# DavidPetrus/ood_object_detection

Hardware: AMD Instinct MI355X
Metric: images/sec, tf_efficientdet_d0 640px bf16 inference + OOD score (DetBenchPredict end-to-end) (higher is better)
Workload: dtype bf16; 1 GPU; tf_efficientdet_d0 640x640 batch=64/GPU C=90, DetBenchPredict: backbone+BiFPN+heads+OOD energy/max-logit+top-k(5000)+decode+hard NMS; global_batch=64, parallelism=image-sharded dp1, no collective, weights=seeded reference init, randomised BN stats, class bias 0, launch=hipgraph, images_in_flight=192

## Files before the change

### include/effdet_hip.h

```cpp
#ifndef EFFDET_HIP_H
#define EFFDET_HIP_H

#ifdef __cplusplus
extern "C" {
#endif

#define EFFDET_F32 0
#define EFFDET_BF16 1
#define EFFDET_BF16X2 2
#define EFFDET_PAD_SYMMETRIC (1 << 24)

int effdet_abi_version(void);
const char* effdet_last_error(void);
int effdet_device_error(int clear);


int effdet_stem_conv(void* stream, int in_dtype, int out_dtype, const void* X, const float* Wt,
                     const float* scale, const float* shift, void* Y, int B, int H, int W, int Cout);

int effdet_stem_dw_fused(void* stream, int in_dtype, int dtype, const void* X, const void* Wk,
                         const float* s1, const float* t1, const float* taps, const float* s2, const float* t2,
                         void* Y, float* pool_partial, int B, int H, int W, int C);
int effdet_stem_dw_parts(int dtype, int H, int W, int C);

int effdet_resize_pad_u8(void* stream, const unsigned char* src, int h, int w, unsigned char* dst, int S, int sw, int sh,
                         const int* bounds_x, const int* coef_x, int ksize_x,
                         const int* bounds_y, const int* coef_y, int ksize_y,
                         const int* fill_rgb, unsigned char* workspace);
int effdet_normalize_u8(void* stream, int out_dtype, const unsigned char* X, const float* mean, const float* stdv,
                        void* Y, int B, int C, long long hw);

typedef struct EffdetResampleDesc {
    const unsigned char* src;
    int h, w;
    int flip_h, flip_v;
    int cx0, cy0, cw, ch;
    int filter;
    int sw, sh;
    int ox, oy;
    int reserved;
} EffdetResampleDesc;
int effdet_resample_batch_u8(void* stream, const EffdetResampleDesc* desc, const EffdetResampleDesc* desc_host, int B,
                             unsigned char* dst, long long dst_image_stride, int S, const int* fill_rgb);

typedef struct EffdetBoxParams {
    float img_w, img_h;
    int flip_h, flip_v;
    float pre_y, pre_x, scale, post_y, post_x, clip_h, clip_w;
    int reserved;
} EffdetBoxParams;
int effdet_transform_boxes(void* stream, const float* boxes, const long long* classes, const EffdetBoxParams* params,
                           int B, int Mmax, float* out_boxes, long long* out_classes, int* counts, unsigned char* valid);
int effdet_stem_conv_u8(void* stream, int out_dtype, const unsigned char* X, const float* mean, const float* stdv,
                        const float* Wt, const float* scale, const float* shift, void* Y, int B, int H, int W, int Cout);
int effdet_stem_dw_fused_u8(void* stream, int dtype, const unsigned char* X, const float* mean, const float* stdv,
                            const void* Wk, const float* s1, const float* t1, const float* taps, const float* s2, const float* t2,
                            void* Y, float* pool_partial, int B, int H, int W, int C);

int effdet_pw_gemm_bn_act(void* stream, int dtype, const void* A, long long M, int K, const void* W, int N,
                          const float* scale, const float* shift, int act, const void* residual,
                          const float* gate, int rows_per_image,
                          void* C, long long c_image_stride, long long ldc);
int effdet_pw_gemm_group(void* stream, int dtype, int n, const void* const* A, const long long* M, const int* K,
                         const void* const* W, const int* N, const float* const* scale, const float* const* shift,
                         int act, void* const* C);

int effdet_dwconv_bn_act(void* stream, int dtype, const void* X, void* Y, const float* Wt,
                         const float* scale, const float* shift, int act, float* pool_partial,
                         int B, int H, int W, int C, int k, int stride);
int effdet_dwconv_blocks_per_image(int Ho, int Wo, int C);

int effdet_mbconv_expand_dw(void* stream, int dtype, const void* X, void* Y, const void* W1,
                            const float* s1, const float* t1, const float* taps,
                            const float* s2, const float* t2, float* pool_partial,
                            int B, int H, int W, int Cin, int mid, int k, int stride);
int effdet_mbconv_tiles_per_image(int dtype, int H, int W, int Cin, int mid, int k, int stride);
int effdet_mbconv_expand_dw_gated(void* stream, int dtype, const void* X, const float* in_gate, void* Y, const void* W1,
                                  const float* s1, const float* t1, const float* taps,
                                  const float* s2, const float* t2, float* pool_partial,
                                  int B, int H, int W, int Cin, int mid, int k, int stride);
int effdet_mbconv_gated_tiles_per_image(int dtype, int H, int W, int Cin, int mid, int k, int stride);
#define EFFDET_MBCONV_PLAN_INTS 17
int effdet_mbconv_plan_describe(int dtype, int H, int W, int Cin, int mid, int k, int stride, int gated, int* out, int n);

int effdet_se_gate(void* stream, const float* partial, int nblk, int hw, const float* W1, const float* b1,
                   const float* W2t, const float* b2, float* gate, int B, int C, int R);


int effdet_maxpool_same(void* stream, int dtype, const void* X, long long x_image_stride,
                        void* Y, long long y_image_stride, int B, int H, int W, int C);

int effdet_sepconv_fused(void* stream, int dtype, int B, int nlevels, const int* level_hw, int n_in,
                         const void* const* in_ptr, const long long* in_image_stride, const int* in_hw,
                         const int* in_mode, int fuse_mode, const float* fuse_w, float fuse_den, int pre_act,
                         const float* dw_w, const void* pw_w, const float* scale, const float* shift,
                         const int* affine_row, int post_act, int F, int N,
                         void* const* out_ptr, const long long* out_image_stride,
                         int ood_classes, int num_anchors, float* ood_energy, float* ood_maxlogit,
                         long long ood_image_stride, const long long* ood_level_off);

int effdet_sepconv_meta(void* stream, int dtype, int B, int nlevels, const int* level_hw,
                        const void* const* in_ptr, const long long* in_image_stride,
                        const float* in_scale, const float* in_shift, const int* in_affine_row, int pre_act,
                        const float* dw_w, const void* pw_w, const float* bias, int F, int N,
                        void* const* out_ptr, const long long* out_image_stride,
                        float* stat_partial, void* const* dw_out, const long long* dw_out_image_stride);
int effdet_sepconv_tiles(int dtype, int nlevels, const int* level_hw, int* level_tile_begin);
int effdet_bn_batch_stats(void* stream, int dtype, const float* partial, int B, int nlevels, const int* level_hw, int N,
                          const float* weight, const float* bias, const int* param_row, float eps,
                          float* out_scale, float* out_shift);


long long effdet_topk_workspace_bytes(int B, long long n_anchors);
int effdet_topk_select(void* stream, int dtype, const void* cls_all, const float* anchor_max, int B, long long n_anchors, int C,
                       const void* box_all, int k, void* out_cls, void* out_box,
                       long long* out_indices, long long* out_classes, void* workspace, long long workspace_bytes);

int effdet_decode_threshold(void* stream, int dtype, const void* cls_topk, const void* box_topk,
                            const float* anchors, const long long* indices, const long long* classes,
                            const float* img_scale, const float* img_size, int B, int k,
                            float* boxes, float* scores, int* classes_out, int* src, int* count, float* maxcoord);
int effdet_decode_threshold_gather(void* stream, int dtype, const void* cls_topk, const void* box_all, long long n_anchors,
                                   const float* anchors, const long long* indices, const long long* classes,
                                   const float* img_scale, const float* img_size, int B, int k,
                                   float* boxes, float* scores, int* classes_out, int* src, int* count, float* maxcoord);

int effdet_nms_hard(void* stream, const float* boxes, const float* scores, const int* classes, const int* src,
                    const int* count, const float* maxcoord, int B, int k, double iou_threshold, int max_det,
                    const float* img_scale, float* det, int* det_count, int* keep_src);

int effdet_detections_hard(void* stream, int dtype, const void* cls_topk, const void* box, long long n_anchors,
                           const float* anchors, const long long* indices, const long long* classes,
                           const float* img_scale_clip, const float* img_size, int B, int k,
                           float* boxes, float* scores, int* classes_out, int* src, int* count, float* maxcoord,
                           double iou_threshold, int max_det, const float* img_scale_out,
                           float* det, int* det_count, int* keep_src);

int effdet_nms_soft(void* stream, const float* boxes, const float* scores, const int* classes, const int* src,
                    const int* count, const float* maxcoord, int B, int k, int method_gaussian, float sigma,
                    float iou_threshold, float score_threshold, int max_det,
                    const float* img_scale, float* det, int* det_count, int* keep_src);

int effdet_nms_soft_large(void* stream, const float* boxes, const float* scores, const int* classes, const int* src,
                          const int* count, const float* maxcoord, int B, int k, int method_gaussian, float sigma,
                          float iou_threshold, float score_threshold, int max_det,
// ... 345 lines not shown
```

### ood_object_detection_amd/_lib.py

```python
import ctypes
import os
import subprocess

_HERE = os.path.dirname(os.path.abspath(__file__))
LIB_PATH = os.path.join(_HERE, 'libeffdet_hip.so')
CSRC = os.path.join(_HERE, 'csrc')

_lib = None

LABEL_PAD = -2 ** 63

c_void_p, c_int, c_ll, c_float, c_double = ctypes.c_void_p, ctypes.c_int, ctypes.c_longlong, ctypes.c_float, ctypes.c_double
P = ctypes.POINTER

SIGNATURES = {
    'effdet_abi_version': (c_int, []),
    'effdet_last_error': (ctypes.c_char_p, []),
    'effdet_device_error': (c_int, [c_int]),
    'effdet_stem_conv': (c_int, [c_void_p, c_int, c_int, c_void_p, c_void_p, c_void_p, c_void_p, c_void_p,
                                 c_int, c_int, c_int, c_int]),
    'effdet_stem_dw_fused': (c_int, [c_void_p, c_int, c_int, c_void_p, c_void_p, c_void_p, c_void_p, c_void_p, c_void_p,
                                     c_void_p, c_void_p, c_void_p, c_int, c_int, c_int, c_int]),
    'effdet_resize_pad_u8': (c_int, [c_void_p, c_void_p, c_int, c_int, c_void_p, c_int, c_int, c_int, c_void_p, c_void_p, c_int,
                                     c_void_p, c_void_p, c_int, c_void_p, c_void_p]),
    'effdet_resample_batch_u8': (c_int, [c_void_p, c_void_p, c_void_p, c_int, c_void_p, c_ll, c_int, c_void_p]),
    'effdet_transform_boxes': (c_int, [c_void_p, c_void_p, c_void_p, c_void_p, c_int, c_int, c_void_p, c_void_p, c_void_p, c_void_p]),
    'effdet_normalize_u8': (c_int, [c_void_p, c_int, c_void_p, c_void_p, c_void_p, c_void_p, c_int, c_int, c_ll]),
    'effdet_stem_conv_u8': (c_int, [c_void_p, c_int, c_void_p, c_void_p, c_void_p, c_void_p, c_void_p, c_void_p, c_void_p,
                                    c_int, c_int, c_int, c_int]),
    'effdet_stem_dw_fused_u8': (c_int, [c_void_p, c_int, c_void_p, c_void_p, c_void_p, c_void_p, c_void_p, c_void_p, c_void_p,
                                        c_void_p, c_void_p, c_void_p, c_void_p, c_int, c_int, c_int, c_int]),
    'effdet_stem_dw_parts': (c_int, [c_int, c_int, c_int, c_int]),
    'effdet_pw_gemm_bn_act': (c_int, [c_void_p, c_int, c_void_p, c_ll, c_int, c_void_p, c_int, c_void_p, c_void_p,
                                      c_int, c_void_p, c_void_p, c_int, c_void_p, c_ll, c_ll]),
    'effdet_pw_gemm_group': (c_int, [c_void_p, c_int, c_int, P(c_void_p), P(c_ll), P(c_int), P(c_void_p), P(c_int), P(c_void_p),
                                     P(c_void_p), c_int, P(c_void_p)]),
    'effdet_dwconv_bn_act': (c_int, [c_void_p, c_int, c_void_p, c_void_p, c_void_p, c_void_p, c_void_p, c_int,
                                     c_void_p, c_int, c_int, c_int, c_int, c_int, c_int]),
    'effdet_dwconv_blocks_per_image': (c_int, [c_int, c_int, c_int]),
    'effdet_mbconv_gated_tiles_per_image': (c_int, [c_int, c_int, c_int, c_int, c_int, c_int, c_int]),
    'effdet_mbconv_expand_dw_gated': (c_int, [c_void_p, c_int, c_void_p, c_void_p, c_void_p, c_void_p, c_void_p, c_void_p, c_void_p,
                                              c_void_p, c_void_p, c_void_p, c_int, c_int, c_int, c_int, c_int, c_int, c_int]),
    'effdet_mbconv_expand_dw': (c_int, [c_void_p, c_int, c_void_p, c_void_p, c_void_p, c_void_p, c_void_p, c_void_p,
                                        c_void_p, c_void_p, c_void_p, c_int, c_int, c_int, c_int, c_int, c_int, c_int]),
    'effdet_mbconv_tiles_per_image': (c_int, [c_int, c_int, c_int, c_int, c_int, c_int, c_int]),
    'effdet_mbconv_plan_describe': (c_int, [c_int, c_int, c_int, c_int, c_int, c_int, c_int, c_int, P(c_int), c_int]),
    'effdet_se_gate': (c_int, [c_void_p, c_void_p, c_int, c_int, c_void_p, c_void_p, c_void_p, c_void_p,
                               c_void_p, c_int, c_int, c_int]),
    'effdet_maxpool_same': (c_int, [c_void_p, c_int, c_void_p, c_ll, c_void_p, c_ll, c_int, c_int, c_int, c_int]),
    'effdet_sepconv_fused': (c_int, [c_void_p, c_int, c_int, c_int, P(c_int), c_int,
                                     P(c_void_p), P(c_ll), P(c_int), P(c_int), c_int, P(c_float), c_float, c_int,
                                     c_void_p, c_void_p, c_void_p, c_void_p, P(c_int), c_int, c_int, c_int,
                                     P(c_void_p), P(c_ll), c_int, c_int, c_void_p, c_void_p, c_ll, P(c_ll)]),
    'effdet_weighted_median': (c_int, [c_void_p, c_void_p, c_void_p, c_int, c_int, c_void_p, c_void_p]),
    'effdet_sqnorm_workspace_floats': (c_ll, []),
    'effdet_sqnorm': (c_int, [c_void_p, c_void_p, c_ll, c_void_p, c_void_p, c_int]),
    'effdet_adam_clip_step': (c_int, [c_void_p, c_void_p, c_void_p, c_void_p, c_void_p, c_ll, c_float, c_float, c_float, c_float,
                                      c_int, c_float, c_void_p]),
    'effdet_adam_clip_step_dev': (c_int, [c_void_p, c_void_p, c_void_p, c_void_p, c_void_p, c_ll, c_float, c_float, c_float, c_float,
                                          c_void_p, c_float, c_void_p]),
    'effdet_group_piece_floats': (c_ll, []),
    'effdet_group_norms': (c_int, [c_void_p, c_void_p, c_ll, c_void_p, c_int, c_int, c_void_p, c_int, c_void_p, c_int, c_void_p, c_int,
                                   c_void_p, c_void_p]),
    'effdet_group_step': (c_int, [c_void_p, c_int, c_void_p, c_void_p, c_void_p, c_void_p, c_ll, c_void_p, c_int, c_int, c_void_p, c_int,
                                  c_void_p, c_int, c_void_p, c_int, c_void_p, c_void_p, c_void_p, c_void_p]),
    'effdet_novelty_score': (c_int, [c_void_p, c_void_p, c_void_p, c_void_p, c_int, c_int, c_int, c_float, c_float, c_int,
                                     c_void_p, c_void_p, c_void_p]),
    'effdet_ood_image_score': (c_int, [c_void_p, c_void_p, c_int, c_ll, c_void_p]),
    'effdet_auroc_counts': (c_int, [c_void_p, c_void_p, c_void_p, c_int, c_int, c_void_p]),
    'effdet_ood_eval_workspace_bytes': (c_ll, [c_ll, c_ll]),
    'effdet_ood_eval_sort_tile': (c_int, []),
    'effdet_ood_eval_sorted_offset': (c_ll, [c_ll, c_ll, c_int]),
    'effdet_ood_eval_append': (c_int, [c_void_p, c_void_p, c_ll, c_ll, c_int, c_int, c_void_p, c_int, c_void_p, c_ll, c_ll, c_float,
                                       c_int, c_void_p, c_ll, c_void_p, c_void_p, c_ll]),
    'effdet_ood_eval_sort': (c_int, [c_void_p, c_void_p, c_ll, c_void_p, c_ll, c_void_p, c_void_p, c_ll]),
    'effdet_ood_eval_metrics': (c_int, [c_void_p, c_ll, c_ll, c_void_p, c_void_p, c_ll, c_double, c_void_p]),
    'effdet_feature_ood_workspace_bytes': (c_ll, [c_ll, c_int]),
    'effdet_feature_ood_fit': (c_int, [c_void_p, c_int, c_int, P(c_void_p), P(c_ll), P(c_ll), P(c_ll), P(c_ll), c_int, c_int, c_int, c_int,
                                       c_ll, c_void_p, c_void_p, c_int, c_ll, c_ll, c_ll, c_void_p, c_int, c_void_p, c_void_p, c_void_p,
                                       c_void_p, c_ll]),
    'effdet_feature_ood_score': (c_int, [c_void_p, c_int, c_int, P(c_void_p), P(c_ll), P(c_ll), P(c_ll), P(c_ll), c_int, c_int, c_int,
                                         c_int, c_ll, c_void_p, c_void_p, c_int, c_void_p, c_void_p, c_void_p, c_void_p, c_void_p,
                                         c_void_p, c_void_p, c_void_p]),
    'effdet_feature_knn_workspace_bytes': (c_ll, [c_ll, c_int, c_int, c_int]),
    'effdet_feature_knn_append': (c_int, [c_void_p, c_int, c_int, P(c_void_p), P(c_ll), P(c_ll), P(c_ll), P(c_ll), c_int, c_int, c_int, c_int,
                                          c_ll, c_void_p, c_void_p, c_int, c_ll, c_ll, c_ll, c_void_p, c_int, c_int, c_ll, c_ll, c_void_p,
                                          c_void_p, c_void_p, c_void_p, c_void_p, c_ll]),
    'effdet_feature_knn_score': (c_int, [c_void_p, c_int, c_int, P(c_void_p), P(c_ll), P(c_ll), P(c_ll), P(c_ll), c_int, c_int, c_int,
                                         c_ll, c_void_p, c_void_p, c_int, c_int, c_int, c_int, c_ll, c_void_p, c_void_p, c_void_p,
                                         c_void_p, c_void_p, c_void_p, c_void_p, c_ll]),
    'effdet_feature_subspace_score': (c_int, [c_void_p, c_int, c_int, P(c_void_p), P(c_ll), P(c_ll), P(c_ll), P(c_ll), c_int, c_int, c_int,
                                              c_ll, c_void_p, c_void_p, c_int, c_void_p, c_void_p, c_void_p, c_int, c_void_p, c_ll, c_ll,
                                              c_int, c_float, c_void_p, c_void_p, c_void_p]),
    'effdet_feature_subspace_calibrate': (c_int, [c_void_p, c_int, c_int, P(c_void_p), P(c_ll), P(c_ll), P(c_ll), P(c_ll), c_int, c_int,
                                                  c_int, c_ll, c_void_p, c_void_p, c_int, c_void_p, c_void_p, c_int, c_void_p, c_ll, c_ll,
                                                  c_int, c_void_p, c_void_p, c_void_p, c_ll]),
    'effdet_feature_subspace_workspace_bytes': (c_ll, [c_ll]),
    'effdet_logit_ood_score': (c_int, [c_void_p, c_int, c_void_p, c_ll, c_ll, c_int, c_int, c_ll, c_ll, c_void_p, c_void_p, c_int, c_float,
                                       c_float, c_int, c_void_p, c_void_p, c_void_p, c_void_p, c_void_p, c_void_p, c_void_p, c_void_p,
                                       c_void_p, c_void_p, c_void_p, c_void_p]),
    'effdet_logit_ood_fit': (c_int, [c_void_p, c_int, c_void_p, c_ll, c_ll, c_int, c_int, c_ll, c_ll, c_void_p, c_void_p, c_int, c_float,
                                     c_int, c_float, c_void_p, c_void_p, c_void_p, c_void_p, c_void_p, c_ll]),
    'effdet_logit_ood_workspace_bytes': (c_ll, [c_ll, c_int]),
    'effdet_energy_reg': (c_int, [c_void_p, c_int, c_void_p, c_void_p, c_int, c_ll, c_int, c_int, c_int, c_float, c_float, c_float,
                                  c_float, c_float, c_int, c_float, c_void_p, c_void_p, c_void_p, c_void_p, c_void_p, c_void_p,
                                  c_void_p, c_ll]),
    'effdet_energy_reg_workspace_bytes': (c_ll, [c_ll]),
    'effdet_sepconv_meta': (c_int, [c_void_p, c_int, c_int, c_int, c_void_p, c_void_p, c_void_p, c_void_p, c_void_p, c_void_p, c_int,
                                    c_void_p, c_void_p, c_void_p, c_int, c_int, c_void_p, c_void_p, c_void_p, c_void_p, c_void_p]),
    'effdet_sepconv_tiles': (c_int, [c_int, c_int, c_void_p, c_void_p]),
    'effdet_bn_batch_stats': (c_int, [c_void_p, c_int, c_void_p, c_int, c_int, c_void_p, c_int, c_void_p, c_void_p, c_void_p, c_float,
                                      c_void_p, c_void_p]),
    'effdet_topk_workspace_bytes': (c_ll, [c_int, c_ll]),
    'effdet_topk_select': (c_int, [c_void_p, c_int, c_void_p, c_void_p, c_int, c_ll, c_int, c_void_p, c_int, c_void_p, c_void_p,
                                   c_void_p, c_void_p, c_void_p, c_ll]),
    'effdet_decode_threshold_gather': (c_int, [c_void_p, c_int, c_void_p, c_void_p, c_ll, c_void_p, c_void_p, c_void_p,
                                               c_void_p, c_void_p, c_int, c_int, c_void_p, c_void_p, c_void_p, c_void_p, c_void_p, c_void_p]),
# ... 202 lines not shown
```

### ood_object_detection_amd/csrc/pw_gemm.hip

```cpp
#include "common.h"

namespace {

struct PwArgs {
    const void* A; long long M; int K;
    const void* W; int N;
    const float* scale; const float* shift; int act;
    const void* res;
    const float* gate; int rows_per_image;
    void* C; long long c_image_stride; long long ldc;
    int tiles_per_image, n_tiles, vec_ok;
};

template <int V> struct PwInt { static constexpr int value = V; };

constexpr int PW_PIX = 128;

template <typename T, int BN, int PT, int NTH, bool GATED>
DEV void pw_gemm_body(const PwArgs& p, const int bid) {
    constexpr bool PAIR = IsPair<T>::value;
    constexpr int KCH = PAIR ? 1 : 2;
    constexpr int EPC = VecTraits<T>::EPC;
    constexpr int KPC = OpGeom<T>::KPC;
    constexpr int PB = OpGeom<T>::PIECE, CB = OpGeom<T>::CHUNK;
    constexpr int NT = BN / 16, NP = NT / 2;
    static_assert(NT % 2 == 0, "tile pairs");
    constexpr int PF = 2;
    constexpr int ROWB = KCH * CB + 16;
    constexpr int W_BYTES = BN * ROWB;
    __shared__ __attribute__((aligned(16))) char lds[2 * W_BYTES];
    extern __shared__ __attribute__((aligned(16))) float gate_lds[];

    const int tid = threadIdx.x, lane = tid & 63, wave = tid >> 6;
    const int frow = lane & 15, fpiece = lane >> 4;
    const int K = p.K, N = p.N;
    const int nt = bid % p.n_tiles;
    const int mt = bid / p.n_tiles;
    const int img = mt / p.tiles_per_image;
    const int pix0 = (mt - img * p.tiles_per_image) * PW_PIX;
    const int n0 = nt * BN;
    const int n_count = (N - n0) < BN ? (N - n0) : BN;
    const long long pitch = (long long)K * (long long)sizeof(T);
    const int nkc = (K + KPC - 1) / KPC;
    const int nst = (nkc + KCH - 1) / KCH;
    const int kbytes = K * (int)sizeof(T);

    const char* arow[PT];
    int pix[PT];
    bool pix_ok[PT];
#pragma unroll
    for (int i = 0; i < PT; ++i) {
        pix[i] = pix0 + 16 * PT * wave + 16 * i + frow;
        pix_ok[i] = pix[i] < p.rows_per_image;
        const long long m = (long long)img * p.rows_per_image + (pix_ok[i] ? pix[i] : 0);
        arow[i] = reinterpret_cast<const char*>(p.A) + m * pitch;
    }
    Frag<T> areg[PF + 1][KCH][PT];
    auto a_load = [&](int stg, int slot) {
#pragma unroll
        for (int sub = 0; sub < KCH; ++sub) {
            const int off = (stg * KCH + sub) * CB + fpiece * PB;
            const int offc = off < kbytes ? off : 0;
#pragma unroll
            for (int i = 0; i < PT; ++i) areg[slot][sub][i] = ld_frag<T>(arow[i] + offc);
        }
    };

    const char* Wb = reinterpret_cast<const char*>(p.W);
    const float* gate = GATED ? p.gate + (long long)img * K : nullptr;
    constexpr int PPR = KCH * 4;
    constexpr int W_PER_THREAD = (BN * PPR + NTH - 1) / NTH;
    auto lds_row = [](int co) { return 16 * (2 * (co >> 5) + ((co >> 2) & 1)) + 4 * ((co >> 3) & 3) + (co & 3); };
    constexpr int WV = PB / 16;
    u32x4 w_reg[W_PER_THREAD][WV];
    if constexpr (GATED) {
        for (int k = tid * 4; k < K; k += NTH * 4) *reinterpret_cast<f32x4*>(gate_lds + k) = *reinterpret_cast<const f32x4*>(gate + k);
    }
    auto w_load = [&](int stg) {
#pragma unroll
        for (int q = 0; q < W_PER_THREAD; ++q) {
            const int idx = tid + NTH * q < BN * PPR ? tid + NTH * q : BN * PPR - 1;
            const int co = idx / PPR, piece = idx % PPR;
            const int ke = stg * KCH * KPC + piece * EPC;
// ... 77 lines not shown
    int stg = 0;
    for (; stg + PF + 1 <= nst; stg += PF + 1) {
        stage(stg, PwInt<0>{});
        stage(stg + 1, PwInt<1>{});
        stage(stg + 2, PwInt<2>{});
    }
    if (stg < nst) {
        stage(stg, PwInt<0>{});
        if (stg + 1 < nst) stage(stg + 1, PwInt<1>{});
    }

    T* Cb = reinterpret_cast<T*>(p.C) + (long long)img * p.c_image_stride;
    const T* Rb = reinterpret_cast<const T*>(p.res);
#pragma unroll
    for (int J = 0; J < NP; ++J) {
        if (J < njp) {
            const int cb = 32 * J + 8 * fpiece;
            const int nvalid = n_count - cb;
            if (nvalid > 0) {
                float sc[8], sh[8];
#pragma unroll
                for (int e = 0; e < 8; ++e) {
                    const int n = n0 + cb + (e < nvalid ? e : 0);
                    sc[e] = p.scale ? p.scale[n] : 1.0f;
                    sh[e] = p.shift[n];
                }
#pragma unroll
                for (int i = 0; i < PT; ++i) {
                    if (!pix_ok[i]) continue;
                    float v[8];
#pragma unroll
                    for (int r = 0; r < 4; ++r) {
                        v[r] = fmaf(acc[i][2 * J][r], sc[r], sh[r]);
                        v[4 + r] = fmaf(acc[i][2 * J + 1][r], sc[4 + r], sh[4 + r]);
                    }
                    if (p.act == 1) {
#pragma unroll
                        for (int e = 0; e < 8; ++e) v[e] = silu_t<T>(v[e]);
                    } else if (p.act == 2) {
#pragma unroll
                        for (int e = 0; e < 8; ++e) v[e] = fmaxf(v[e], 0.f);
                    }
                    T* dst = Cb + (long long)pix[i] * p.ldc + n0 + cb;
                    if (Rb != nullptr) {
                        const T* rsrc = Rb + ((long long)img * p.rows_per_image + pix[i]) * N + n0 + cb;
                        if (p.vec_ok && nvalid >= 8) {
                            const F8 rv = load8<T>(rsrc);
#pragma unroll
                            for (int e = 0; e < 8; ++e) v[e] += rv.v[e];
                        } else if constexpr (!PAIR) {
#pragma unroll
                            for (int e = 0; e < 8; ++e) if (e < nvalid) v[e] += to_f<T>(rsrc[e]);
                        }
                    }
                    if (p.vec_ok && nvalid >= 8) {
                        F8 o;
#pragma unroll
                        for (int e = 0; e < 8; ++e) o.v[e] = v[e];
                        store8<T>(dst, o);
                    } else if constexpr (!PAIR) {
#pragma unroll
                        for (int e = 0; e < 8; ++e) if (e < nvalid) dst[e] = from_f<T>(v[e]);
                    }
                }
            }
        }
    }
}

template <typename T, int BN, int PT, int NTH, bool GATED>
__global__ __launch_bounds__(NTH, 2) void pw_gemm_kernel(PwArgs p) {
    pw_gemm_body<T, BN, PT, NTH, GATED>(p, blockIdx.x);
}

constexpr int PW_GROUP_MAX = 8;
struct PwGroupArgs { int n; int first[PW_GROUP_MAX + 1]; PwArgs p[PW_GROUP_MAX]; };

template <typename T, int BN, int PT, int NTH>
__global__ __launch_bounds__(NTH, 2) void pw_gemm_group_kernel(PwGroupArgs g) {
    int i = 0;
#pragma unroll
    for (int q = 1; q < PW_GROUP_MAX; ++q) if (q < g.n && (int)blockIdx.x >= g.first[q]) i = q;
    pw_gemm_body<T, BN, PT, NTH, false>(g.p[i], (int)blockIdx.x - g.first[i]);
}

template <typename T>
int pw_prepare(PwArgs& a, int& bn, long long& blocks) {
    int ntl = (a.N + 191) / 192;
    bn = ((a.N + ntl - 1) / ntl + 31) / 32 * 32;
    a.tiles_per_image = (a.rows_per_image + PW_PIX - 1) / PW_PIX;
    const long long images = a.M / a.rows_per_image;
    a.n_tiles = (a.N + bn - 1) / bn;
    blocks = images * a.tiles_per_image * a.n_tiles;
    if (blocks <= 0 || blocks > 0x7fffffffLL) return EFFDET_EINVAL;
    const size_t esz = sizeof(T);
    a.vec_ok = ((size_t)a.N * esz) % 16 == 0 && ((size_t)a.ldc * esz) % 16 == 0 && ((size_t)a.c_image_stride * esz) % 16 == 0 &&
               reinterpret_cast<uintptr_t>(a.C) % 16 == 0 && (a.res == nullptr || reinterpret_cast<uintptr_t>(a.res) % 16 == 0);
    return EFFDET_OK;
}

template <typename T>
int launch_pw_group(hipStream_t st, PwGroupArgs& g) {
    int bn0 = 0;
    long long total = 0;
    for (int i = 0; i < g.n; ++i) {
        int bn; long long blocks;
        const int rc = pw_prepare<T>(g.p[i], bn, blocks);
        if (rc) return rc;
        if (i == 0) bn0 = bn; else if (bn != bn0) return EFFDET_EINVAL;
        g.first[i] = (int)total;
        total += blocks;
        if (total > 0x7fffffffLL) return EFFDET_EINVAL;
    }
    g.first[g.n] = (int)total;
    dim3 grid((unsigned)total);
    const bool small = total < 512;
#define PWG_LAUNCH(BN_) do { if (small && BN_ != 128) hipLaunchKernelGGL((pw_gemm_group_kernel<T, BN_ == 128 ? 96 : BN_, 1, 512>), grid, dim3(512), 0, st, g); \
                             else hipLaunchKernelGGL((pw_gemm_group_kernel<T, BN_, 2, 256>), grid, dim3(256), 0, st, g); } while (0)
    switch (bn0) {
        case 32:  PWG_LAUNCH(32); break;
        case 64:  PWG_LAUNCH(64); break;
        case 96:  PWG_LAUNCH(96); break;
        default: return EFFDET_EINVAL;
    }
#undef PWG_LAUNCH
    return effdet_check_launch();
}

template <typename T>
int launch_pw(hipStream_t st, PwArgs& a) {
    int bn; long long blocks;
    const int rc0 = pw_prepare<T>(a, bn, blocks);
    if (rc0) return rc0;
    dim3 grid((unsigned)blocks);
    const bool small = blocks < 512;
    const bool gated = a.gate != nullptr;
    const size_t dyn = gated ? ((size_t)a.K * 4 + 15) / 16 * 16 : 0;
#define PW_LAUNCH_G(BN_, G_) do { if (small && BN_ != 128) hipLaunchKernelGGL((pw_gemm_kernel<T, BN_ == 128 ? 96 : BN_, 1, 512, G_>), grid, dim3(512), dyn, st, a);  \
                            else hipLaunchKernelGGL((pw_gemm_kernel<T, BN_, 2, 256, G_>), grid, dim3(256), dyn, st, a); } while (0)
#define PW_LAUNCH(BN_) do { if (gated) PW_LAUNCH_G(BN_, true); else PW_LAUNCH_G(BN_, false); } while (0)
    switch (bn) {
        case 32:  PW_LAUNCH(32); break;
        case 64:  PW_LAUNCH(64); break;
        case 96:  PW_LAUNCH(96); break;
        case 128: PW_LAUNCH(128); break;
        case 160: PW_LAUNCH(160); break;
        case 192: PW_LAUNCH(192); break;
        default: return EFFDET_EINVAL;
    }
#undef PW_LAUNCH
#undef PW_LAUNCH_G
    return effdet_check_launch();
}

}

extern "C" int effdet_pw_gemm_bn_act(void* stream, int dtype,
                                     const void* A, long long M, int K,
                                     const void* W, int N,
                                     const float* scale, const float* shift, int act,
                                     const void* residual,
                                     const float* gate, int rows_per_image,
                                     void* C, long long c_image_stride, long long ldc) {
    EFFDET_ENTER();
    if (!A || !W || !C || !shift || M <= 0 || K <= 0 || N <= 0) return EFFDET_EINVAL;
    if (K % 8 != 0 || M > 0x7fffffffLL) return EFFDET_EINVAL;
    if (act < 0 || act > 2) return EFFDET_EINVAL;
    if (rows_per_image <= 0) { rows_per_image = (int)(M > 0x7fffffffLL ? 0x7fffffff : M); }
    if ((M % rows_per_image) != 0) return EFFDET_EINVAL;
    if (ldc <= 0) ldc = N;
    if (c_image_stride <= 0) c_image_stride = (long long)rows_per_image * ldc;
    PwArgs a{A, M, K, W, N, scale, shift, act, residual, gate, rows_per_image, C, c_image_stride, ldc, 0, 0, 0};
    hipStream_t st = reinterpret_cast<hipStream_t>(stream);
    if (dtype == 0) return launch_pw<float>(st, a);
    if (dtype == 1) return launch_pw<bf16_t>(st, a);
    if (dtype == 2) {
        if (N % 8 || ldc % 8 || c_image_stride % 8 || reinterpret_cast<uintptr_t>(A) % 32 || reinterpret_cast<uintptr_t>(W) % 32 ||
            reinterpret_cast<uintptr_t>(C) % 32 || (residual && reinterpret_cast<uintptr_t>(residual) % 32)) return EFFDET_EINVAL;
        return launch_pw<bf16p_t>(st, a);
    }
    return EFFDET_EINVAL;
}

extern "C" int effdet_pw_gemm_group(void* stream, int dtype, int n, const void* const* A, const long long* M, const int* K,
                                    const void* const* W, const int* N, const float* const* scale, const float* const* shift,
                                    int act, void* const* C) {
    EFFDET_ENTER();
    if (n < 1 || n > PW_GROUP_MAX || !A || !M || !K || !W || !N || !scale || !shift || !C || act < 0 || act > 2) return EFFDET_EINVAL;
    PwGroupArgs g;
    g.n = n;
    for (int i = 0; i < n; ++i) {
        if (!A[i] || !W[i] || !C[i] || !shift[i] || M[i] <= 0 || M[i] > 0x7fffffffLL || K[i] <= 0 || K[i] % 8 || N[i] <= 0) return EFFDET_EINVAL;
        g.p[i] = PwArgs{A[i], M[i], K[i], W[i], N[i], scale[i], shift[i], act, nullptr, nullptr, (int)M[i], C[i], M[i] * N[i], N[i], 0, 0, 0};
    }
    hipStream_t st = reinterpret_cast<hipStream_t>(stream);
    if (dtype == 0) return launch_pw_group<float>(st, g);
    if (dtype == 1) return launch_pw_group<bf16_t>(st, g);
    if (dtype == 2) {
        for (int i = 0; i < n; ++i)
            if (N[i] % 8 || reinterpret_cast<uintptr_t>(A[i]) % 32 || reinterpret_cast<uintptr_t>(W[i]) % 32 || reinterpret_cast<uintptr_t>(C[i]) % 32)
                return EFFDET_EINVAL;
        return launch_pw_group<bf16p_t>(st, g);
    }
    return EFFDET_EINVAL;
}
```

Baseline: 17000 images/sec.

## Add weight-stationary pointwise GEMM kernel for gated projections with cost-model planner

Adds a weight-stationary pointwise GEMM in which each wave keeps a 16-channel slice of the weights in registers, pre-multiplied by the SE gate. Activation slabs are streamed through double-buffered LDS into MFMA 16x16x32 bf16. A heuristic planner chooses the variant, the channel split and the row-sharing geometry, and routes gated bf16 projections to the new form by default. The aim is to stop reloading weights and reapplying the gate per tile in SE-gated projection convs. In exchange it adds register pressure, large LDS use and an unvalidated cost model.

```diff
diff --git a/include/effdet_hip.h b/include/effdet_hip.h
--- a/include/effdet_hip.h
+++ b/include/effdet_hip.h
@@ -61,6 +61,12 @@
                           const float* scale, const float* shift, int act, const void* residual,
                           const float* gate, int rows_per_image,
                           void* C, long long c_image_stride, long long ldc);
+int effdet_pw_gemm_bn_act_form(void* stream, int dtype, const void* A, long long M, int K, const void* W, int N,
+                               const float* scale, const float* shift, int act, const void* residual,
+                               const float* gate, int rows_per_image,
+                               void* C, long long c_image_stride, long long ldc, int form);
+#define EFFDET_PW_GEMM_PLAN_INTS 10
+int effdet_pw_gemm_plan_describe(int dtype, int K, int N, int rows_per_image, int gated, int residual, int* out, int n);
 int effdet_pw_gemm_group(void* stream, int dtype, int n, const void* const* A, const long long* M, const int* K,
                          const void* const* W, const int* N, const float* const* scale, const float* const* shift,
                          int act, void* const* C);
diff --git a/ood_object_detection_amd/_lib.py b/ood_object_detection_amd/_lib.py
--- a/ood_object_detection_amd/_lib.py
+++ b/ood_object_detection_amd/_lib.py
@@ -33,6 +33,9 @@
     'effdet_stem_dw_parts': (c_int, [c_int, c_int, c_int, c_int]),
     'effdet_pw_gemm_bn_act': (c_int, [c_void_p, c_int, c_void_p, c_ll, c_int, c_void_p, c_int, c_void_p, c_void_p,
                                       c_int, c_void_p, c_void_p, c_int, c_void_p, c_ll, c_ll]),
+    'effdet_pw_gemm_bn_act_form': (c_int, [c_void_p, c_int, c_void_p, c_ll, c_int, c_void_p, c_int, c_void_p, c_void_p,
+                                           c_int, c_void_p, c_void_p, c_int, c_void_p, c_ll, c_ll, c_int]),
+    'effdet_pw_gemm_plan_describe': (c_int, [c_int, c_int, c_int, c_int, c_int, c_int, P(c_int), c_int]),
     'effdet_pw_gemm_group': (c_int, [c_void_p, c_int, c_int, P(c_void_p), P(c_ll), P(c_int), P(c_void_p), P(c_int), P(c_void_p),
                                      P(c_void_p), c_int, P(c_void_p)]),
     'effdet_dwconv_bn_act': (c_int, [c_void_p, c_int, c_void_p, c_void_p, c_void_p, c_void_p, c_void_p, c_int,
diff --git a/ood_object_detection_amd/csrc/pw_gemm.hip b/ood_object_detection_amd/csrc/pw_gemm.hip
--- a/ood_object_detection_amd/csrc/pw_gemm.hip
+++ b/ood_object_detection_amd/csrc/pw_gemm.hip
@@ -1,4 +1,5 @@
 #include "common.h"
+#include <math.h>
 
 namespace {
 
@@ -242,6 +243,283 @@
 #pragma unroll
     for (int q = 1; q < PW_GROUP_MAX; ++q) if (q < g.n && (int)blockIdx.x >= g.first[q]) i = q;
     pw_gemm_body<T, BN, PT, NTH, false>(g.p[i], (int)blockIdx.x - g.first[i]);
+}
+
+struct PwWsArgs {
+    PwArgs a;
+    int nkc, ppr, xpitch, slab_bytes;
+    int share_tiles, nshare, nsplit, split_tiles;
+    int units, vec4_ok;
+    FastDiv fd_ppr;
+};
+
+template <int NKC, int SPT, int NPL, int MINW>
+__global__ __launch_bounds__(512, MINW) void pw_ws_kernel(PwWsArgs q) {
+    extern __shared__ __attribute__((aligned(16))) char ws_lds[];
+    const PwArgs& p = q.a;
+    const int tid = threadIdx.x, nth = blockDim.x, lane = tid & 63;
+    const int wave = __builtin_amdgcn_readfirstlane(tid >> 6);
+    const int frow = lane & 15, kg = lane >> 4;
+    const int rr = blockIdx.x >> 3;
+    const int unit = (rr / q.nsplit) * 8 + (blockIdx.x & 7);
+    if (unit >= q.units) return;
+    const int split = rr % q.nsplit;
+    const int img = unit / q.nshare;
+    const int rows = p.rows_per_image;
+    const int tile0 = (unit - img * q.nshare) * q.share_tiles;
+    const int tiles_img = (rows + 15) >> 4;
+    const int tile_end = tile0 + q.share_tiles < tiles_img ? tile0 + q.share_tiles : tiles_img;
+    if (tile0 >= tile_end) return;
+    const int K = p.K, N = p.N, kbytes = K * 2;
+    const int c0 = 16 * (split * q.split_tiles + wave);
+    const bool active = c0 < N;
+
+    for (int i = tid * 16; i < 2 * q.slab_bytes; i += nth * 16) *reinterpret_cast<u32x4*>(ws_lds + i) = u32x4{0u, 0u, 0u, 0u};
+    __syncthreads();
+
+    bf16x8 wf[NKC];
+    float* const gate_s = reinterpret_cast<float*>(ws_lds + 2 * q.slab_bytes);
+    float* const aff_s = gate_s + NKC * 32;
+    {
+        const bool nok = c0 + frow < N;
+        const char* wrow = reinterpret_cast<const char*>(p.W) + (long long)(nok ? c0 + frow : 0) * kbytes;
+#pragma unroll
+        for (int c = 0; c < NKC; ++c) {
+            const int off = c * 64 + kg * 16;
+            const bool kin = c * 64 < kbytes - kg * 16;
+            const unsigned keep = (nok && kin) ? 0xFFFFFFFFu : 0u;
+            const u32x4 raw = *reinterpret_cast<const u32x4*>(wrow + (kin ? off : 0)) & u32x4{keep, keep, keep, keep};
+            wf[c] = __builtin_bit_cast(bf16x8, raw);
+        }
+        if (p.gate != nullptr) {
+            const float* gate = p.gate + (long long)img * K;
+            for (int k = tid * 4; k < NKC * 32; k += nth * 4)
+                *reinterpret_cast<f32x4*>(gate_s + k) = k < K ? *reinterpret_cast<const f32x4*>(gate + k) : f32x4{0.f, 0.f, 0.f, 0.f};
+        }
+        for (int i = tid; i < 16 * (nth >> 6); i += nth) {
+            const int n = 16 * split * q.split_tiles + i < N ? 16 * split * q.split_tiles + i : N - 1;
+            aff_s[i] = p.scale ? p.scale[n] : 1.0f;
+            aff_s[16 * (nth >> 6) + i] = p.shift[n];
+        }
+    }
+
+    const char* Ab = reinterpret_cast<const char*>(p.A) + (long long)img * rows * kbytes;
+    const int total = SPT * 16 * q.ppr;
+    u32x4 sreg[NPL];
+    auto slab_load = [&](int tile) {
+        const char* base = Ab + (long long)tile * 16 * kbytes;
+        const int left = rows - tile * 16;
+        if (left >= SPT * 16) {
+#pragma unroll
+            for (int j = 0; j < NPL; ++j) {
+                const int i = tid + nth * j;
+                sreg[j] = *reinterpret_cast<const u32x4*>(base + (unsigned)((i < total ? i : total - 1) * 16));
+            }
+        } else {
+            const int limit = left * q.ppr;
+#pragma unroll
+            for (int j = 0; j < NPL; ++j) {
+                const int i = tid + nth * j;
+                sreg[j] = *reinterpret_cast<const u32x4*>(base + (unsigned)((i < limit ? i : 0) * 16));
+            }
+        }
+    };
+    auto slab_store = [&](int buf) {
+        char* dst = ws_lds + buf * q.slab_bytes;
+#pragma unroll
+        for (int j = 0; j < NPL; ++j) {
+            const int i0 = tid + nth * j, i = i0 < total ? i0 : total - 1;
+            const int px = fdiv(i, q.fd_ppr);
+            *reinterpret_cast<u32x4*>(dst + px * q.xpitch + (i - px * q.ppr) * 16) = sreg[j];
+        }
+    };
+
+    const int ch = c0 + 4 * kg;
+    const int nvalid = N - ch;
+    const float* const sc_s = aff_s + 16 * wave + 4 * kg;
+    const float* const sh_s = sc_s + 16 * (nth >> 6);
+    bf16_t* Cb = reinterpret_cast<bf16_t*>(p.C) + (long long)img * p.c_image_stride;
+    const bf16_t* Rb = reinterpret_cast<const bf16_t*>(p.res);
+    const int blane = frow * q.xpitch + kg * 16;
+
+    slab_load(tile0);
+    slab_store(0);
+    __syncthreads();
+    if (p.gate != nullptr) {
+#pragma unroll
+        for (int c = 0; c < NKC; ++c) {
+            const float* gp = gate_s + c * 32 + kg * 8;
+            const f32x4 g0 = *reinterpret_cast<const f32x4*>(gp), g1 = *reinterpret_cast<const f32x4*>(gp + 4);
+#pragma unroll
+            for (int e = 0; e < 8; ++e) wf[c][e] = (bf16_t)((float)wf[c][e] * (e < 4 ? g0[e] : g1[e - 4]));
+            if (c % 2 == 1) __builtin_amdgcn_sched_barrier(0);
+        }
+    }
+    const bool res4 = Rb != nullptr && q.vec4_ok;
+    int buf = 0;
+    for (int tile = tile0; tile < tile_end; tile += SPT, buf ^= 1) {
+        const bool more = tile + SPT < tile_end;
+        u32x2 rres[SPT];
+        if (res4) {
+#pragma unroll
+            for (int t = 0; t < SPT; ++t) {
+                const int pix = (tile + t) * 16 + frow;
+                rres[t] = *reinterpret_cast<const u32x2*>(Rb + ((long long)img * rows + (pix < rows ? pix : rows - 1)) * N + (nvalid >= 4 ? ch : 0));
+            }
+        }
+        if (more) slab_load(tile + SPT);
+        f32x4 acc[SPT];
+#pragma unroll
+        for (int t = 0; t < SPT; ++t) acc[t] = f32x4{0.f, 0.f, 0.f, 0.f};
+        if (active) {
+            const char* xs = ws_lds + buf * q.slab_bytes + blane;
+#pragma unroll
+            for (int c = 0; c < NKC; ++c) {
+#pragma unroll
+                for (int t = 0; t < SPT; ++t) {
+                    const bf16x8 xf = *reinterpret_cast<const bf16x8*>(xs + t * 16 * q.xpitch + c * 64);
+                    acc[t] = __builtin_amdgcn_mfma_f32_16x16x32_bf16(wf[c], xf, acc[t], 0, 0, 0);
+                }
+                if ((c + 1) % (4 / SPT) == 0) __builtin_amdgcn_sched_barrier(0);
+            }
+        }
+        if (more) slab_store(buf ^ 1);
+        if (active) {
+#pragma unroll
+            for (int t = 0; t < SPT; ++t) {
+                const int pix = (tile + t) * 16 + frow;
+                if (tile + t < tile_end && pix < rows && nvalid > 0) {
+                    const f32x4 sc = *reinterpret_cast<const f32x4*>(sc_s), sh = *reinterpret_cast<const f32x4*>(sh_s);
+                    float v[4];
+#pragma unroll
+                    for (int r = 0; r < 4; ++r) v[r] = fmaf(acc[t][r], sc[r], sh[r]);
+                    if (p.act == 1) {
+#pragma unroll
+                        for (int r = 0; r < 4; ++r) v[r] = silu_t<bf16_t>(v[r]);
+                    } else if (p.act == 2) {
+#pragma unroll
+                        for (int r = 0; r < 4; ++r) v[r] = fmaxf(v[r], 0.f);
+                    }
+                    bf16_t* dst = Cb + (long long)pix * p.ldc + ch;
+                    if (Rb != nullptr) {
+                        if (q.vec4_ok && nvalid >= 4) {
+                            const bf16x4 rv = __builtin_bit_cast(bf16x4, rres[t]);
+#pragma unroll
+                            for (int r = 0; r < 4; ++r) v[r] += (float)rv[r];
+                        } else {
+                            const bf16_t* rsrc = Rb + ((long long)img * rows + pix) * N + ch;
+#pragma unroll
+                            for (int r = 0; r < 4; ++r) if (r < nvalid) v[r] += (float)rsrc[r];
+                        }
+                    }
+                    if (q.vec4_ok && nvalid >= 4) {
+                        store4<bf16_t>(dst, v[0], v[1], v[2], v[3]);
+                    } else {
+#pragma unroll
+                        for (int r = 0; r < 4; ++r) if (r < nvalid) dst[r] = (bf16_t)v[r];
+                    }
+                }
+            }
+        }
+        __syncthreads();
+    }
+}
+
+typedef void (*PwWsKernel)(PwWsArgs);
+struct PwWsVariant { int nkc, spt, npl, minw; PwWsKernel kern; };
+#define PW_WS_V(NKC_, SPT_, NPL_, MINW_) {NKC_, SPT_, NPL_, MINW_, pw_ws_kernel<NKC_, SPT_, NPL_, MINW_>}
+const PwWsVariant PW_WS_VARIANTS[] = {
+    PW_WS_V(8, 1, 4, 4), PW_WS_V(16, 1, 4, 4), PW_WS_V(21, 1, 4, 3), PW_WS_V(36, 1, 8, 2),
+};
+#undef PW_WS_V
+constexpr int PW_WS_NVARIANTS = (int)(sizeof(PW_WS_VARIANTS) / sizeof(PW_WS_VARIANTS[0]));
+constexpr int PW_WS_LDS_MAX = 160 * 1024;
+
+struct PwWsGeometry { int variant, nkc, spt, npl, ppr, xpitch, slab_bytes, lds, share_tiles, nshare, nsplit, waves; };
+
+PwWsGeometry pick_ws(int K, int N, int rows) {
+    PwWsGeometry g{};
+    g.variant = -1;
+    if (K <= 0 || K % 8 || N <= 0 || rows <= 0) return g;
+    const int nkc = (K + 31) / 32, ppr = K / 8;
+    const int ntiles = (N + 15) / 16, tiles_img = (rows + 15) / 16;
+    int v = 0;
+    while (v < PW_WS_NVARIANTS && PW_WS_VARIANTS[v].nkc < nkc) ++v;
+    if (v == PW_WS_NVARIANTS) return g;
+    const PwWsVariant& pv = PW_WS_VARIANTS[v];
+    const int xpitch = pv.nkc * 64 + 32;
+    const int slab_bytes = pv.spt * 16 * xpitch;
+    const int lds = 2 * slab_bytes + pv.nkc * 128 + 2 * 16 * 8 * 4;
+    if (lds > PW_WS_LDS_MAX) return g;
+    double best = -1.0;
+    for (int nsplit = (ntiles + 7) / 8; nsplit <= ntiles && nsplit <= (ntiles + 7) / 8 + 2; ++nsplit) {
+        const int waves = (ntiles + nsplit - 1) / nsplit;
+        if ((nsplit - 1) * waves >= ntiles) continue;
+        int per_cu = 4 * pv.minw / waves;
+        if (per_cu > PW_WS_LDS_MAX / lds) per_cu = PW_WS_LDS_MAX / lds;
+        if (per_cu < 1) continue;
+        if ((pv.spt * 16 * ppr + waves * 64 - 1) / (waves * 64) > pv.npl) continue;
+        for (int nshare = 1; nshare <= tiles_img; ++nshare) {
+            const int share = (tiles_img + nshare - 1) / nshare;
+            if ((nshare - 1) * share >= tiles_img) continue;
+            if (share < 10 && nshare > 1) break;
+            const long long wgs = 64LL * nsplit * nshare;
+            const int L = (int)((wgs + 255) / 256);
+            const int conc = L < per_cu ? L : per_cu;
+            const double slab = 16.0 * pv.spt * K * 2;
+            const double tau = slab / 15000.0 > 1.2 ? slab / 15000.0 : 1.2;
+            const double alone = (share + pv.spt - 1) / pv.spt * tau + 3.0;
+            const double shared = conc * (16.0 * share + 16.0 * waves) * K * 2 / 23000.0;
+            double cost = (double)((L + per_cu - 1) / per_cu) * (alone > shared ? alone : shared);
+            if (wgs < 256) cost *= sqrt(256.0 / (double)wgs);
+            if (best < 0 || cost < best * 0.999) {
+                best = cost;
+                g = PwWsGeometry{v, nkc, pv.spt, pv.npl, ppr, xpitch, slab_bytes, lds, share, nshare, nsplit, waves};
+            }
+        }
+    }
+    return g;
+}
+
+enum PwForm { PW_STREAMING = 1, PW_STATIONARY = 2 };
+struct PwPlan { int form; int bn, n_tiles; PwWsGeometry ws; };
+
+PwPlan pw_plan(int K, int N, int rows_per_image, bool gated, bool residual, int dtype) {
+    (void)residual;
+    PwPlan p{};
+    const int ntl = (N + 191) / 192;
+    p.bn = ((N + ntl - 1) / ntl + 31) / 32 * 32;
+    p.n_tiles = (N + p.bn - 1) / p.bn;
+    p.form = PW_STREAMING;
+    p.ws.variant = -1;
+    if (dtype != 1) return p;
+    p.ws = pick_ws(K, N, rows_per_image);
+    if (p.ws.variant >= 0 && gated && p.bn >= 64 && (PW_WS_VARIANTS[p.ws.variant].minw >= 3 || (p.ws.nkc > 24 && p.n_tiles > 1))) p.form = PW_STATIONARY;
+    return p;
+}
+
+int launch_pw_ws(hipStream_t st, const PwArgs& a, const PwWsGeometry& g) {
+    if (g.variant < 0) return EFFDET_EINVAL;
+    if (reinterpret_cast<uintptr_t>(a.A) % 16 || reinterpret_cast<uintptr_t>(a.W) % 16 || (a.gate && reinterpret_cast<uintptr_t>(a.gate) % 16))
+        return EFFDET_EINVAL;
+    PwWsArgs q{};
+    q.a = a;
+    q.nkc = g.nkc; q.ppr = g.ppr; q.xpitch = g.xpitch; q.slab_bytes = g.slab_bytes;
+    q.share_tiles = g.share_tiles; q.nshare = g.nshare; q.nsplit = g.nsplit; q.split_tiles = g.waves;
+    const long long images = a.M / a.rows_per_image;
+    const long long units = images * g.nshare, blocks = (units + 7) / 8 * 8 * g.nsplit;
+    if (units > 0x7fffffffLL || blocks > 0x7fffffffLL) return EFFDET_EINVAL;
+    q.units = (int)units;
+    q.vec4_ok = a.N % 4 == 0 && a.ldc % 4 == 0 && a.c_image_stride % 4 == 0 && reinterpret_cast<uintptr_t>(a.C) % 8 == 0 &&
+                (a.res == nullptr || reinterpret_cast<uintptr_t>(a.res) % 8 == 0);
+    q.fd_ppr = make_fastdiv(g.ppr);
+    const PwWsKernel kern = PW_WS_VARIANTS[g.variant].kern;
+    if (g.lds > 64 * 1024) {
+        if (hipFuncSetAttribute(reinterpret_cast<const void*>(kern), hipFuncAttributeMaxDynamicSharedMemorySize, PW_WS_LDS_MAX) != hipSuccess)
+            return EFFDET_ELAUNCH;
+    }
+    hipLaunchKernelGGL(kern, dim3((unsigned)blocks), dim3(g.waves * 64), g.lds, st, q);
+    return effdet_check_launch();
 }
 
 template <typename T>
@@ -315,6 +593,35 @@
 
 }
 
+extern "C" int effdet_pw_gemm_bn_act_form(void* stream, int dtype,
+                                          const void* A, long long M, int K,
+                                          const void* W, int N,
+                                          const float* scale, const float* shift, int act,
+                                          const void* residual,
+                                          const float* gate, int rows_per_image,
+                                          void* C, long long c_image_stride, long long ldc, int form) {
+    EFFDET_ENTER();
+    if (!A || !W || !C || !shift || M <= 0 || K <= 0 || N <= 0) return EFFDET_EINVAL;
+    if (K % 8 != 0 || M > 0x7fffffffLL) return EFFDET_EINVAL;
+    if (act < 0 || act > 2) return EFFDET_EINVAL;
+    if (form < 0 || form > 2) return EFFDET_EINVAL;
+    if (rows_per_image <= 0) { rows_per_image = (int)(M > 0x7fffffffLL ? 0x7fffffff : M); }
+    if ((M % rows_per_image) != 0) return EFFDET_EINVAL;
+    if (ldc <= 0) ldc = N;
+    if (c_image_stride <= 0) c_image_stride = (long long)rows_per_image * ldc;
+    PwArgs a{A, M, K, W, N, scale, shift, act, residual, gate, rows_per_image, C, c_image_stride, ldc, 0, 0, 0};
+    hipStream_t st = reinterpret_cast<hipStream_t>(stream);
+    if (dtype < 0 || dtype > 2) return EFFDET_EINVAL;
+    const PwPlan plan = pw_plan(K, N, rows_per_image, gate != nullptr, residual != nullptr, dtype);
+    if (form == 0) form = plan.form;
+    if (form == PW_STATIONARY) return launch_pw_ws(st, a, plan.ws);
+    if (dtype == 0) return launch_pw<float>(st, a);
+    if (dtype == 1) return launch_pw<bf16_t>(st, a);
+    if (N % 8 || ldc % 8 || c_image_stride % 8 || reinterpret_cast<uintptr_t>(A) % 32 || reinterpret_cast<uintptr_t>(W) % 32 ||
+        reinterpret_cast<uintptr_t>(C) % 32 || (residual && reinterpret_cast<uintptr_t>(residual) % 32)) return EFFDET_EINVAL;
+    return launch_pw<bf16p_t>(st, a);
+}
+
 extern "C" int effdet_pw_gemm_bn_act(void* stream, int dtype,
                                      const void* A, long long M, int K,
                                      const void* W, int N,
@@ -322,24 +629,24 @@
                                      const void* residual,
                                      const float* gate, int rows_per_image,
                                      void* C, long long c_image_stride, long long ldc) {
-    EFFDET_ENTER();
-    if (!A || !W || !C || !shift || M <= 0 || K <= 0 || N <= 0) return EFFDET_EINVAL;
-    if (K % 8 != 0 || M > 0x7fffffffLL) return EFFDET_EINVAL;
-    if (act < 0 || act > 2) return EFFDET_EINVAL;
-    if (rows_per_image <= 0) { rows_per_image = (int)(M > 0x7fffffffLL ? 0x7fffffff : M); }
-    if ((M % rows_per_image) != 0) return EFFDET_EINVAL;
-    if (ldc <= 0) ldc = N;
-    if (c_image_stride <= 0) c_image_stride = (long long)rows_per_image * ldc;
-    PwArgs a{A, M, K, W, N, scale, shift, act, residual, gate, rows_per_image, C, c_image_stride, ldc, 0, 0, 0};
-    hipStream_t st = reinterpret_cast<hipStream_t>(stream);
-    if (dtype == 0) return launch_pw<float>(st, a);
-    if (dtype == 1) return launch_pw<bf16_t>(st, a);
-    if (dtype == 2) {
-        if (N % 8 || ldc % 8 || c_image_stride % 8 || reinterpret_cast<uintptr_t>(A) % 32 || reinterpret_cast<uintptr_t>(W) % 32 ||
-            reinterpret_cast<uintptr_t>(C) % 32 || (residual && reinterpret_cast<uintptr_t>(residual) % 32)) return EFFDET_EINVAL;
-        return launch_pw<bf16p_t>(st, a);
-    }
-    return EFFDET_EINVAL;
+    return effdet_pw_gemm_bn_act_form(stream, dtype, A, M, K, W, N, scale, shift, act, residual, gate, rows_per_image, C, c_image_stride, ldc, 0);
+}
+
+extern "C" int effdet_pw_gemm_plan_describe(int dtype, int K, int N, int rows_per_image, int gated, int residual, int* out, int n) {
+    if (!out || n <= 0 || dtype < 0 || dtype > 2 || K <= 0 || K % 8 || N <= 0 || rows_per_image <= 0) return EFFDET_EINVAL;
+    const PwPlan p = pw_plan(K, N, rows_per_image, gated != 0, residual != 0, dtype);
+    int v[EFFDET_PW_GEMM_PLAN_INTS] = {0};
+    v[0] = p.form;
+    if (p.form == PW_STREAMING) {
+        v[1] = p.bn; v[2] = p.n_tiles; v[3] = PW_PIX;
+    } else {
+        const PwWsGeometry& g = p.ws;
+        v[1] = PW_WS_VARIANTS[g.variant].nkc; v[2] = 16 * g.spt; v[3] = g.share_tiles; v[4] = g.nshare; v[5] = g.nsplit;
+        v[6] = g.waves; v[7] = g.lds; v[8] = g.xpitch; v[9] = g.npl;
+    }
+    const int m = n < EFFDET_PW_GEMM_PLAN_INTS ? n : EFFDET_PW_GEMM_PLAN_INTS;
+    for (int i = 0; i < m; ++i) out[i] = v[i];
+    return m;
 }
 
 extern "C" int effdet_pw_gemm_group(void* stream, int dtype, int n, const void* const* A, const long long* M, const int* K,
```

Measured after the change: 17270 images/sec (median of 4 runs). 1.6% higher.
